# GithinjiHans/LZZX-NeRF

Measured on AMD Instinct MI355X. Metric: rendered samples/s (512x512 triplane head, max_steps 192), higher is better.
Workload: dtype f32

## Files before the change

### lzzx_nerf_amd/csrc/lz_frame.hip

```cpp
#include <stdlib.h>

#include "lz_march.h"
#include "lz_head_slice.h"
#include "lz_head_f16_slice.h"
#include "lz_head_f16w_slice.h"

#ifndef LZF_WG
#define LZF_WG 1024
#endif
#define LZF_WAVES (LZF_WG / 64)
#define LZF_BINS 256
#define LZF_LUT 256
#define LZF_MARCH_PROBES 2
#define LZF_Q_HEAD 0
#define LZF_Q_SIZE 1
#define LZF_DONE 3
#define LZF_SAMPLES 5
#define LZF_ITER 6
#define LZF_ROWS 72
#define LZF_P_HEAD 8
#define LZF_P_SIZE 9
#define LZF_CEFF 10
#define LZF_SCHED_K 11
#define LZF_TICKET 12
#define LZF_CAP_MAX_STEPS 4096
#define LZF_HIST 128
#define LZF_CURSOR 384

struct LzFrameK {
    const float* rays_o; const float* rays_d; const uint8_t* grid; const float* aabb;
    float* nears; float* fars; float* rays_t;
    int* order; int* state; uint8_t* keys;
    float* weights_sum; float* depth; float* image; float* amb0_sum; float* amb1_sum; float* unc_sum;
    float* out; const float* bg; uint8_t* out_rgb24; int* ray_counts;
    float bg_scalar, bound, dt_gamma, T_thresh, min_near;
    uint32_t N, max_steps, C, H;
    const float* noises;
    const float* occ;
    float* t_end;
    int* ray_last;
    int* cap_ws;
    uint32_t cap_mode, phase2, N_total;
    LzMarchFrame mf;
};

typedef const char __attribute__((address_space(4))) lz_kernarg_t;
struct LzfOut {
    lz_kernarg_t* f;
    template <typename T> __device__ __forceinline__ T get(size_t off) const {
        return *reinterpret_cast<const volatile T __attribute__((address_space(4)))*>(f + off);
    }
};
#define LZF_OUT(o, name) ((o).template get<decltype(LzFrameK::name)>(__builtin_offsetof(LzFrameK, name)))
static_assert(alignof(LzFrameK) == 8 && __is_trivially_copyable(LzFrameK), "LZF_OUT reads LzFrameK from the kernel-argument segment at round8(ARGS_BEFORE)");
template <size_t ARGS_BEFORE>
__device__ __forceinline__ LzfOut lzf_out() {
    return LzfOut{(lz_kernarg_t*)__builtin_amdgcn_kernarg_segment_ptr() + ((ARGS_BEFORE + 7) & ~size_t(7))};
}

__device__ __forceinline__ void lzf_write_pixel(const LzfOut& O, int ray, float ws, float d, float r, float g, float b, float a0, float a1,
                                                float u, int cnt) {
    LZF_OUT(O, weights_sum)[ray] = ws;
    LZF_OUT(O, depth)[ray] = d;
    const float rgb[3] = {r, g, b};
    float* image = LZF_OUT(O, image);
    float* out = LZF_OUT(O, out);
// ... 89 lines not shown
            const int v = (bin && threadIdx.x + off < LZF_BINS) ? start[threadIdx.x + off] : 0;
            __syncthreads();
            if (bin) start[threadIdx.x] += v;
            __syncthreads();
        }
        const int incl = bin ? start[threadIdx.x] : 0;
        __syncthreads();
        if (bin) start[threadIdx.x] = incl - h;
        if (blockIdx.x == 0 && threadIdx.x == 1) { F.state[LZF_Q_SIZE] = incl; F.state[LZF_DONE] = 1; F.state[LZF_ITER] = 1; }
    }
    __syncthreads();
    const uint32_t n = blockIdx.x * blockDim.x + threadIdx.x;
    const int key = n < F.N ? (int)F.keys[n] : 0;
    const int lrank = key > 0 ? atomicAdd(&lcount[key], 1) : 0;
    __syncthreads();
    if (bin && threadIdx.x > 0) {
        const int c = lcount[threadIdx.x];
        if (c > 0) lbase[threadIdx.x] = atomicAdd(F.state + LZF_CURSOR + threadIdx.x, c);
    }
    __syncthreads();
    if (key > 0) F.order[start[key] + lbase[key] + lrank] = (int)n;
}

enum { SF_RAY = 0, SF_T, SF_FAR, SF_DT, SF_WS, SF_D, SF_R, SF_G, SF_B, SF_A0, SF_A1, SF_U, SF_CNT,
       SF_SH };
template <int PREC, int S, int ROWS> struct LzfFields {
    static constexpr int SH_WORDS = PREC == 1 ? 8 : 16;
    static constexpr int ST = SF_SH + SH_WORDS;
    static constexpr int X = ST, Y = ST + 1, Z = ST + 2, TS = ST + 3;
    static constexpr int OSIG = S > 1 ? ST + 4 : ST, OR = OSIG + 1, OG = OSIG + 2, OB = OSIG + 3, OA0 = OSIG + 4, OA1 = OSIG + 5, OU = OSIG + 6;
    static constexpr int IT = OSIG + 7;
    static constexpr int RD = S > 1 ? ST + 12 : (ROWS > 1 ? ST + 7 : ST);
    static constexpr bool GEO = ROWS < 3;
    static constexpr int COUNT = RD + 3 + (GEO ? 6 : 0);
};

struct LzShFromSlot {
    const float* slot;
    int ls, ns;
    __device__ __forceinline__ void prepare() const {}
    __device__ __forceinline__ float comp_iq(int i, int q) const { return slot[(SF_SH + 4 * i + q) * ns + ls]; }
    __device__ __forceinline__ float comp_qj(int q, int j) const { return slot[(SF_SH + 4 * q + j) * ns + ls]; }
};
struct LzShFromSlot16 {
    const float* slot;
    int ls, ns;
    __device__ __forceinline__ void prepare() const {}
};
__device__ __forceinline__ void w_sh_pk(const LzShFromSlot16& f, int h, uint32_t (&w)[4]) {
#pragma unroll
    for (int k = 0; k < 4; k++) w[k] = __float_as_uint(f.slot[(SF_SH + 4 * h + k) * f.ns + f.ls]);
}
template <int PREC, bool GEO = false>
__device__ __forceinline__ void lzf_store_sh(const float* __restrict__ ro, const float* __restrict__ d, float* slot, int s, int ns, int rd_field) {
    float o[16];
    lz_sh_eval(d[0], d[1], d[2], 4, o, nullptr, nullptr, nullptr);
    slot[rd_field * ns + s] = 1 / d[0];
    slot[(rd_field + 1) * ns + s] = 1 / d[1];
    slot[(rd_field + 2) * ns + s] = 1 / d[2];
    if constexpr (GEO) {
#pragma unroll
        for (int k = 0; k < 3; k++) {
            slot[(rd_field + 3 + k) * ns + s] = ro[k];
            slot[(rd_field + 6 + k) * ns + s] = d[k];
        }
    }
    if constexpr (PREC == 1) {
#pragma unroll
        for (int k = 0; k < 8; k++) slot[(SF_SH + k) * ns + s] = __uint_as_float(h_cvt2(o[2 * k], o[2 * k + 1], false));
    } else {
#pragma unroll
        for (int k = 0; k < 16; k++) slot[(SF_SH + k) * ns + s] = o[k];
    }
}

__device__ __forceinline__ void lzf_slot_take(const LzfOut& O, bool ph2, int ray, float* slot, int* sloti, int sl, int ns) {
    if (__builtin_expect(ph2, 0)) {
        slot[SF_WS * ns + sl] = LZF_OUT(O, weights_sum)[ray];
        slot[SF_D * ns + sl] = LZF_OUT(O, depth)[ray];
        const float* image = LZF_OUT(O, image);
        slot[SF_R * ns + sl] = image[(size_t)ray * 3];
        slot[SF_G * ns + sl] = image[(size_t)ray * 3 + 1];
        slot[SF_B * ns + sl] = image[(size_t)ray * 3 + 2];
        slot[SF_A0 * ns + sl] = LZF_OUT(O, amb0_sum)[ray];
        slot[SF_A1 * ns + sl] = LZF_OUT(O, amb1_sum)[ray];
        slot[SF_U * ns + sl] = LZF_OUT(O, unc_sum)[ray];
        sloti[SF_CNT * ns + sl] = (int)LZF_OUT(O, max_steps);
    } else {
#pragma unroll
        for (int f = SF_WS; f <= SF_U; f++) slot[f * ns + sl] = 0.0f;
        sloti[SF_CNT * ns + sl] = 0;
    }
}
enum { LZF_END_BOX = 0, LZF_END_T = 1, LZF_END_CAP = 2 };
__device__ __forceinline__ void lzf_ray_end(const LzfOut& O, bool ph2, int ray, int kind, int composited, int report, float t, float ws, float d,
                                            float r, float g, float b, float a0, float a1, float u) {
    if (__builtin_expect(LZF_OUT(O, cap_mode) != 0, 0)) {
        report = composited;
        if (kind == LZF_END_T) {
            if (LZF_OUT(O, ray_counts)) { report = -composited; LZF_OUT(O, rays_t)[ray] = t; }
            if (!ph2) LZF_OUT(O, ray_last)[ray] = composited - 1;
        } else if (!ph2) {
            LZF_OUT(O, ray_last)[ray] = composited;
            if (kind == LZF_END_CAP) LZF_OUT(O, rays_t)[ray] = t;
        }
    }
    lzf_write_pixel(O, ray, ws, d, r, g, b, a0, a1, u, report);
}

template <int PREC> struct LzfHead;
template <> struct LzfHead<0> {
    using Args = LzHeadArgs; using Ctx = LzHeadCtx; using Out = LzHeadOut; using ShSlot = LzShFromSlot;
    static constexpr int LDS_WORDS = LzHeadLds<false>::FLOATS;
    __device__ static __forceinline__ void stage(const Args& P, float* lds, int q, Ctx& c) { lz_head_stage<false>(P, lds, LZF_WG, q, c); }
    template <typename ShFn>
    __device__ static __forceinline__ void slice(const Ctx& c, int lane, float x, float y, float z, ShFn f, Out& o) {
        lz_head_slice<false, false, true, true>(c, lane, x, y, z, f, o);
    }
};
template <> struct LzfHead<2> : LzfHead<0> {
    template <typename ShFn>
    __device__ static __forceinline__ void slice(const Ctx& c, int lane, float x, float y, float z, ShFn f, Out& o) {
        lz_head_slice<false, true, true, true>(c, lane, x, y, z, f, o);
    }
};
template <> struct LzfHead<1> {
    using Args = LzHead16Args; using Ctx = LzHead16Ctx; using Out = LzHead16wOut; using ShSlot = LzShFromSlot16;
    static constexpr int LDS_WORDS = LZ_HEAD16W_LDS_H8 * 4;
    __device__ static __forceinline__ void stage(const Args& P, float* lds, int, Ctx& c) { lz_head16w_stage(P, reinterpret_cast<lz_h8*>(lds), LZF_WG, c); }
    template <typename ShFn>
    __device__ static __forceinline__ void slice(const Ctx& c, int lane, float x, float y, float z, ShFn f, Out& o) {
        lz_head16w_slice<true, LZ_F16W_PRIO != 0>(c, lane, x, y, z, f, o);
    }
};

template <int PREC, int S, int ROWS>
__global__ void __launch_bounds__(LZF_WG, LZF_WG / 256)
lz_k_frame(typename LzfHead<PREC>::Args P, LzFrameK F) {
    using HD = LzfHead<PREC>;
    static_assert(PREC == 1 ? ROWS == 2 : (ROWS == 1 || S == 1), "slot rows per wave: f16 two; f32 one, or several with one sample per ray and pass");
    constexpr int NS = 16 * ROWS;
    using FL = LzfFields<PREC, S, ROWS>;
    constexpr int NF = FL::COUNT;
    constexpr int SF_X = FL::X, SF_Y = FL::Y, SF_Z = FL::Z, SF_TS = FL::TS, SF_OSIG = FL::OSIG, SF_OR = FL::OR, SF_OG = FL::OG, SF_OB = FL::OB,
                  SF_OA0 = FL::OA0, SF_OA1 = FL::OA1, SF_OU = FL::OU, SF_IT = FL::IT, SF_RD = FL::RD;
    (void)SF_RD; (void)SF_X; (void)SF_Y; (void)SF_Z; (void)SF_TS; (void)SF_IT; (void)SF_OSIG; (void)SF_OR; (void)SF_OG; (void)SF_OB; (void)SF_OA0; (void)SF_OA1; (void)SF_OU;
    constexpr int SLOT_WORDS = LZF_WAVES * NF * NS;
    __shared__ __align__(16) float lds[HD::LDS_WORDS + SLOT_WORDS + 4 + LZF_LUT];
    const int lane = threadIdx.x & 63, wave = threadIdx.x >> 6;
    const int s = (S > 1) ? (lane & (NS - 1)) : (lane & 15), q = lane >> 4;
    const bool slot_lane = lane < NS;
    static_assert(alignof(typename HD::Args) <= 8, "lz_k_frame(Args P, LzFrameK F): F sits at round8(sizeof(Args)) of the kernel-argument segment");
// ... 130 lines not shown
                            kk = got;
                            if (kk == 0) {
                                const int c0 = sloti[SF_CNT * NS + s];
                                lzf_ray_end(OUT, ph2, ray, LZF_END_BOX, c0, c0, t0, slot[SF_WS * NS + s], slot[SF_D * NS + s], slot[SF_R * NS + s], slot[SF_G * NS + s],
                                            slot[SF_B * NS + s], slot[SF_A0 * NS + s], slot[SF_A1 * NS + s], slot[SF_U * NS + s]);
                                my_samples += c0 - cnt_base;
                                ray = -1;
                                sloti[SF_RAY * NS + s] = -1;
                            }
                        }
                    }
                }
                if (!__ballot(leader && ray < 0 && !dry)) break;
            }
            if (leader) sloti[SF_IT * NS + s] = kk;
            if (!__ballot(kk > 0)) {
                if (dry) break;
                continue;
            }
            const int lkk = sloti[SF_IT * NS + lead];
            const bool live = sloti[SF_RAY * NS + lead] >= 0 && j < lkk;
            const float px = live ? slot[SF_X * NS + s] : 0.0f, py = live ? slot[SF_Y * NS + s] : 0.0f, pz = live ? slot[SF_Z * NS + s] : 0.0f;
            typename HD::Out o;
            HD::slice(ctx, lane, px, py, pz, typename HD::ShSlot{slot, lead, NS}, o);
            my_slices += ROWS;
            if constexpr (PREC == 1) {
                const int hh = lane >> 5;
                slot[(SF_OR + hh) * NS + s] = o.a;
                slot[(hh ? SF_OSIG : SF_OB) * NS + s] = hh ? 1.0f - lz_expf(-o.b * slot[SF_DT * NS + s]) : o.b;
                if (hh == 0) { slot[SF_OA0 * NS + s] = o.ambaud; slot[SF_OA1 * NS + s] = o.eyeatt; slot[SF_OU * NS + s] = o.unc; }
            } else if (q == 0) {
                slot[SF_OSIG * NS + s] = 1.0f - lz_expf(-o.sigma * slot[SF_DT * NS + s]);
                slot[SF_OR * NS + s] = o.rgb[0]; slot[SF_OG * NS + s] = o.rgb[1]; slot[SF_OB * NS + s] = o.rgb[2];
                slot[SF_OA0 * NS + s] = o.ambaud; slot[SF_OA1 * NS + s] = o.eyeatt; slot[SF_OU * NS + s] = o.unc;
            }
            __builtin_amdgcn_wave_barrier();
            if (leader && kk > 0) {
                float ws = slot[SF_WS * NS + s], d = slot[SF_D * NS + s], r = slot[SF_R * NS + s], g = slot[SF_G * NS + s], b = slot[SF_B * NS + s];
                float a0 = slot[SF_A0 * NS + s], a1 = slot[SF_A1 * NS + s], u = slot[SF_U * NS + s], t = slot[SF_T * NS + s];
                int step = 0;
                while (step < kk) {
                    const int sl = s + step;
                    const float alpha = slot[SF_OSIG * NS + sl];
                    const float T = 1 - ws;
                    const float w = alpha * T;
                    ws += w;
                    t = slot[SF_TS * NS + sl];
// ... 81 lines not shown
                        lzf_ray_end(OUT, ph2, ray, LZF_END_BOX, c0, c0, t, slot[SF_WS * NS + sl], slot[SF_D * NS + sl], slot[SF_R * NS + sl], slot[SF_G * NS + sl],
                                    slot[SF_B * NS + sl], slot[SF_A0 * NS + sl], slot[SF_A1 * NS + sl], slot[SF_U * NS + sl]);
                        my_samples += c0 - cnt_base;
                        ray = -1;
                        sloti[SF_RAY * NS + sl] = -1;
                        x = y = z = 0.0f;
                    }
                }
                if (!__ballot(slot_lane && ray < 0 && !dry)) break;
            }
            const unsigned long long have_mask = __ballot(have);
            if (!have_mask) {
                if (dry && !__ballot(slot_lane && ray >= 0)) break;
                continue;
            }
            typename HD::Out o;
            if constexpr (PREC == 1) {
                const int rs = lane & 31, hh = lane >> 5;
                auto lo2 = [](float v) -> float {
                    const auto r = __builtin_amdgcn_permlane32_swap(__float_as_uint(v), __float_as_uint(v), false, false);
                    return __uint_as_float(r[0]);
                };
                const float px = lo2(x), py = lo2(y), pz = lo2(z);
                HD::slice(ctx, lane, px, py, pz, typename HD::ShSlot{slot, rs, NS}, o);
                my_slices += 2;
                slot[(SF_OR + hh) * NS + rs] = o.a;
                slot[(hh ? SF_OSIG : SF_OB) * NS + rs] = o.b;
                if (hh == 0) { slot[SF_OA0 * NS + rs] = o.ambaud; slot[SF_OA1 * NS + rs] = o.eyeatt; slot[SF_OU * NS + rs] = o.unc; }
            } else {
#pragma unroll 1
                for (int row = 0; row < ROWS; row++) {
                    if (ROWS > 1 && !((have_mask >> (16 * row)) & 0xffffull)) continue;
                    const int rs = 16 * row + s;
                    const float px = __shfl(x, rs, 64), py = __shfl(y, rs, 64), pz = __shfl(z, rs, 64);
                    HD::slice(ctx, lane, px, py, pz, typename HD::ShSlot{slot, rs, NS}, o);
                    my_slices++;
                    if (ROWS > 1 && q == 0) {
                        slot[SF_OSIG * NS + rs] = o.sigma;
                        slot[SF_OR * NS + rs] = o.rgb[0]; slot[SF_OG * NS + rs] = o.rgb[1]; slot[SF_OB * NS + rs] = o.rgb[2];
                        slot[SF_OA0 * NS + rs] = o.ambaud; slot[SF_OA1 * NS + rs] = o.eyeatt; slot[SF_OU * NS + rs] = o.unc;
                    }
                }
            }
            __builtin_amdgcn_wave_barrier();
            if (have) {
                float sg, c0, c1, c2, am0, am1, un;
                if constexpr (PREC != 1) { sg = o.sigma; c0 = o.rgb[0]; c1 = o.rgb[1]; c2 = o.rgb[2]; am0 = o.ambaud; am1 = o.eyeatt; un = o.unc; }
                if (ROWS > 1) {
                    sg = slot[SF_OSIG * NS + sl];
                    c0 = slot[SF_OR * NS + sl]; c1 = slot[SF_OG * NS + sl]; c2 = slot[SF_OB * NS + sl];
                    am0 = slot[SF_OA0 * NS + sl]; am1 = slot[SF_OA1 * NS + sl]; un = slot[SF_OU * NS + sl];
                }
                const float dt = slot[SF_DT * NS + sl];
                float ws = slot[SF_WS * NS + sl];
                const float alpha = 1.0f - lz_expf(-sg * dt);
                const float T = 1 - ws;
                const float w = alpha * T;
                ws += w;
// ... 287 lines not shown
    return LZ_OK;
}

static void lzf_level_tables(const lz_head_params* p, float* scale, uint32_t* res) {
    for (int l = 0; l < 12; l++) {
        const float sc = exp2f((float)l * p->S) * (float)p->H - 1.0f;
        scale[l] = sc;
        res[l] = (uint32_t)ceilf(sc) + 1u;
    }
}

static int lzf_fill(const lz_frame_fused* f, LzFrameK& K) {
    K.rays_o = f->rays_o; K.rays_d = f->rays_d; K.grid = f->grid; K.aabb = f->aabb;
    K.nears = f->nears; K.fars = f->fars; K.rays_t = f->rays_t;
    K.order = f->order; K.state = f->state; K.keys = f->keys;
    K.weights_sum = f->weights_sum; K.depth = f->depth; K.image = f->image; K.amb0_sum = f->amb_aud_sum; K.amb1_sum = f->amb_eye_sum;
    K.unc_sum = f->unc_sum; K.out = f->out; K.bg = f->bg; K.out_rgb24 = f->out_rgb24; K.ray_counts = f->ray_counts;
    K.bg_scalar = f->bg_scalar; K.bound = f->bound; K.dt_gamma = f->dt_gamma; K.T_thresh = f->T_thresh; K.min_near = f->min_near;
    K.N = f->N; K.max_steps = f->max_steps; K.C = f->C; K.H = f->H;
    K.noises = f->noises;
    K.occ = f->occupied_aabb; K.t_end = f->t_end;
    K.ray_last = f->ray_last; K.cap_ws = f->cap_ws; K.cap_mode = f->cap_mode; K.phase2 = 0; K.N_total = f->N_total;
    K.mf = lz_march_frame(f->bound, f->max_steps, f->C, f->H);
    return LZ_OK;
}

static int lzf_check(const lz_frame_fused* f, const char* who) {
    const lz_head_params* p = &f->head;
    LZ_REQUIRE(f->rays_o && f->rays_d && f->grid && f->aabb && f->nears && f->fars && f->rays_t && f->order && f->state && f->keys &&
                   f->weights_sum && f->depth && f->image && f->amb_aud_sum && f->amb_eye_sum && f->unc_sum && f->out,
               LZ_ERR_BAD_ARGUMENT, "%s: incomplete lz_frame_fused", who);
    LZ_REQUIRE(p->emb_xy && p->emb_yz && p->emb_xz && p->offsets && p->packed && p->enc_a, LZ_ERR_BAD_ARGUMENT, "%s: incomplete lz_head_params", who);
    LZ_REQUIRE(p->testing, LZ_ERR_UNSUPPORTED, "%s: inference only (head.testing must be 1)", who);
    LZ_REQUIRE(p->precision >= 0 && p->precision <= 2, LZ_ERR_BAD_ARGUMENT, "%s: precision must be 0 (f32), 1 (f16) or 2 (f32, folded geo)", who);
    LZ_REQUIRE(f->C >= 1 && f->C <= 8 && f->H > 0, LZ_ERR_BAD_ARGUMENT, "%s: cascade must be in [1, 8]", who);
    LZ_REQUIRE(!f->occupied_aabb || f->t_end, LZ_ERR_BAD_ARGUMENT, "%s: occupied_aabb needs the t_end scratch buffer", who);
    LZ_REQUIRE(f->cap_mode == LZ_FRAME_CAP_PER_RAY || f->cap_mode == LZ_FRAME_CAP_REFERENCE, LZ_ERR_BAD_ARGUMENT, "%s: cap_mode must be 0 (per ray) or 1 (the reference's schedule)", who);
    if (f->cap_mode == LZ_FRAME_CAP_REFERENCE) {
        LZ_REQUIRE(f->ray_last && f->cap_ws, LZ_ERR_BAD_ARGUMENT, "%s: cap_mode 1 needs the ray_last and cap_ws buffers", who);
        LZ_REQUIRE(f->max_steps <= LZF_CAP_MAX_STEPS, LZ_ERR_UNSUPPORTED, "%s: cap_mode 1 supports max_steps <= %d", who, LZF_CAP_MAX_STEPS);
        LZ_REQUIRE(f->N_total == 0 || f->N_total >= f->N, LZ_ERR_BAD_ARGUMENT, "%s: N_total is the ray count of the whole frame (>= N)", who);
    }
    LZ_REQUIRE(f->bound > 0.0f && f->bound <= p->bound, LZ_ERR_BAD_ARGUMENT,
               "%s: the march's bound must not exceed the head's (the reference uses one `bound` for both, renderer.py:94, network.py:100)", who);
    return LZ_OK;
}
// ... 27 lines not shown
        a.offsets = p->offsets; a.packed = reinterpret_cast<const lz_h8*>(p->packed); a.enc_a = p->enc_a; a.ind_code = p->ind_code;
        a.eye = p->eye; a.bound = p->bound;
        lzf_level_tables(p, a.scale, a.res);
        switch (S) {
            case 1: hipLaunchKernelGGL((lz_k_frame<1, 1, 2>), dim3(grid), dim3(LZF_WG), 0, st, a, K); break;
            case 2: hipLaunchKernelGGL((lz_k_frame<1, 2, 2>), dim3(grid), dim3(LZF_WG), 0, st, a, K); break;
            case 4: hipLaunchKernelGGL((lz_k_frame<1, 4, 2>), dim3(grid), dim3(LZF_WG), 0, st, a, K); break;
            case 8: hipLaunchKernelGGL((lz_k_frame<1, 8, 2>), dim3(grid), dim3(LZF_WG), 0, st, a, K); break;
            default: hipLaunchKernelGGL((lz_k_frame<1, 16, 2>), dim3(grid), dim3(LZF_WG), 0, st, a, K); break;
        }
    } else {
        LzHeadArgs a;
        a.emb[0] = p->emb_xy; a.emb[1] = p->emb_yz; a.emb[2] = p->emb_xz;
        a.offsets = p->offsets; a.packed = reinterpret_cast<const float*>(p->packed); a.enc_a = p->enc_a; a.ind_code = p->ind_code; a.eye = p->eye;
        a.bound = p->bound; a.testing = 1;
        lzf_level_tables(p, a.scale, a.res);
        if (p->precision == 2) { LZF_SWITCH(2) } else { LZF_SWITCH(0) }
    }
#undef LZF_SWITCH
#undef LZF_LAUNCH
    return LZ_OK;
}

extern "C" int lz_frame_finish(const lz_frame_fused* f, lz_stream_t stream) {
    LZ_REQUIRE(f, LZ_ERR_BAD_ARGUMENT, "frame_finish: null");
    LZ_REQUIRE(f->cap_mode == LZ_FRAME_CAP_REFERENCE, LZ_ERR_BAD_ARGUMENT, "frame_finish: only after lz_frame_render with cap_mode 1");
    if (f->N == 0 && f->state) return LZ_OK;
    int rc = lzf_check(f, "frame_finish");
    if (rc != LZ_OK) return rc;
    hipStream_t st = lz_st(stream);
    LzFrameK K;
    lzf_fill(f, K);
    if (f->defer_finish) hipLaunchKernelGGL(lz_k_frame_schedule, dim3(1), dim3(256), LZF_SCHED_LDS_INTS(f->max_steps) * sizeof(int), st, K);
    K.phase2 = 1;
    rc = lzf_launch_persistent(f, K, st);
    if (rc != LZ_OK) return rc;
    if (f->ray_counts) hipLaunchKernelGGL(lz_k_frame_counts, dim3(lz_div_up(f->N, 256)), dim3(256), 0, st, K);
    LZ_CHECK_LAUNCH("frame_finish");
    return LZ_OK;
}

extern "C" int lz_frame_render(const lz_frame_fused* f, lz_timing* timing, lz_stream_t stream) {
    LZ_REQUIRE(f, LZ_ERR_BAD_ARGUMENT, "frame_render: null");
    hipStream_t st = lz_st(stream);
    if (f->N == 0 && f->state) {
        hipError_t e = hipMemsetAsync(f->state, 0, LZ_FRAME_STATE_INTS * sizeof(int32_t), st);
        if (e == hipSuccess && f->cap_mode == LZ_FRAME_CAP_REFERENCE && f->cap_ws) {
            LZ_REQUIRE(f->max_steps <= LZF_CAP_MAX_STEPS, LZ_ERR_UNSUPPORTED, "frame_render: cap_mode 1 supports max_steps <= %d", LZF_CAP_MAX_STEPS);
            e = hipMemsetAsync(f->cap_ws, 0, LZ_FRAME_CAP_WS_INTS((size_t)f->max_steps) * sizeof(int32_t), st);
        }
        if (e != hipSuccess) { lz_set_error("frame_render: memset: %s", hipGetErrorString(e)); return (int)e; }
        return LZ_OK;
    }
    int rc = lzf_check(f, "frame_render");
    if (rc != LZ_OK) return rc;
    LzFrameK K;
    lzf_fill(f, K);
    hipError_t hrc = hipMemsetAsync(f->state, 0, LZ_FRAME_STATE_INTS * sizeof(int32_t), st);
    if (hrc != hipSuccess) { lz_set_error("frame_render: memset: %s", hipGetErrorString(hrc)); return (int)hrc; }
    const bool ref_cap = f->cap_mode == LZ_FRAME_CAP_REFERENCE;
    const uint32_t nb = lz_div_up(f->N, LZF_PREP_WG);
    hipLaunchKernelGGL(lz_k_frame_prepare, dim3(nb), dim3(LZF_PREP_WG), 0, st, K);
    hipLaunchKernelGGL(lz_k_frame_scatter, dim3(nb), dim3(LZF_PREP_WG), 0, st, K);
    if (timing) (void)lz_timing_mark(timing, 0, stream);
    rc = lzf_launch_persistent(f, K, st);
    if (rc != LZ_OK) return rc;
    if (timing) (void)lz_timing_mark(timing, 1, stream);
    if (ref_cap) {
        const size_t lds = LZF_SCHED_LDS_INTS((size_t)f->max_steps) * sizeof(int);
        uint32_t hb = lz_div_up(f->N, 1024 * 8);
        hb = hb < 1 ? 1 : (hb > 32 ? 32 : hb);
        if (f->defer_finish) hipLaunchKernelGGL(lz_k_frame_cap_hist<false>, dim3(hb), dim3(1024), lds, st, K);
        else hipLaunchKernelGGL(lz_k_frame_cap_hist<true>, dim3(hb), dim3(1024), lds, st, K);
    }
    LZ_CHECK_LAUNCH("frame_render");
    if (ref_cap && !f->defer_finish) return lz_frame_finish(f, stream);
    return LZ_OK;
}
```

### lzzx_nerf_amd/csrc/lz_head_gather.h

```cpp
#ifndef LZ_HEAD_GATHER_H
#define LZ_HEAD_GATHER_H
#ifndef LZ_GATHER_PACK16
#define LZ_GATHER_PACK16 false
#endif
#ifndef LZ_GATHER_PACK32
#define LZ_GATHER_PACK32 false
#endif
#include "lz_common.h"
#include "lzzx_detmath.h"

#define LZ_LVTAB_WORDS 128
#define LZ_LVTAB_SCALE 16
#define LZ_LVTAB_STRIDE 32
#define LZ_LVTAB_QUEUE 48
#define LZ_LVTAB_HMUL 49
#define LZ_LVTAB_ENCA 64
#define LZ_LVTAB_MASK 96
#define LZ_LVTAB_ENCA16 108
#define LZ_LVTAB_IND16 124
#define LZ_LVTAB_DENSE0 62

__device__ __forceinline__ void lz_level_table_fill(int* tab, const int* __restrict__ offsets, const float* scale, const uint32_t* res) {
    const uint32_t t = threadIdx.x;
    if (t < 13) tab[t] = offsets[t];
    if (t < 12) {
        const uint32_t hs = (uint32_t)(offsets[t + 1] - offsets[t]), stride = res[t] + 1u;
        const bool dense = stride <= hs && (uint64_t)stride * stride <= hs;
        reinterpret_cast<float*>(tab)[LZ_LVTAB_SCALE + t] = scale[t];
        tab[LZ_LVTAB_STRIDE + t] = dense ? (int)stride : 0;
        tab[LZ_LVTAB_HMUL + t] = dense ? 0 : (int)(2654435761u & 0x00ffffffu);
        tab[LZ_LVTAB_MASK + t] = dense ? -1 : (int)(hs - 1u);
    }
    if (t == 0) {
        tab[LZ_LVTAB_QUEUE] = 0;
        int d0 = 1;
        for (int l = 0; l < 4; l++) {
// ... 144 lines not shown
```

### lzzx_nerf_amd/csrc/lz_head_layers.h

```cpp
#ifndef LZ_HEAD_LAYERS_H
#define LZ_HEAD_LAYERS_H
#include "lz_common.h"
#include "lzzx_detmath.h"

typedef float lz_f4 __attribute__((ext_vector_type(4)));

enum { LZ_L_A1 = 0, LZ_L_A2, LZ_L_E1, LZ_L_S1, LZ_L_S2, LZ_L_S3, LZ_L_C1, LZ_L_U1, LZ_L_COUNT };
constexpr int LZ_KS[LZ_L_COUNT] = {   9, 16,  9, 18, 16, 16, 21,  9 };
constexpr int LZ_NT[LZ_L_COUNT] = {   4,  2,  1,  4,  4,  4,  4,  2 };
constexpr int lz_frag_base(int layer) {
    int b = 0;
    for (int i = 0; i < layer; i++) b += LZ_KS[i] * LZ_NT[i];
    return b;
}
constexpr int lz_kt(int layer) { return (LZ_KS[layer] + 3) / 4; }
constexpr int lz_bfrag_base(int layer) {
    int b = 0;
    for (int i = 0; i < layer; i++) b += i == LZ_L_U1 ? 0 : lz_kt(i) * LZ_NT[i];
    return b;
}
constexpr int LZ_BFRAGS = lz_bfrag_base(LZ_L_COUNT);
constexpr int LZ_FRAGS_INFER = lz_frag_base(LZ_L_U1);
constexpr int LZ_FRAGS_ALL = lz_frag_base(LZ_L_COUNT);
constexpr int LZ_WV_C2 = 0, LZ_WV_SIG = 192, LZ_WV_E2 = 256, LZ_WV_U2 = 272, LZ_WV_FLOATS = 320;
static_assert(LZ_FRAGS_ALL * 64 + LZ_WV_FLOATS == LZ_HEAD_PACKED_FLOATS, "packed size mismatch with the header");


struct LzHeadArgs {
    const float* emb[3];
    const int* offsets;
    const float* packed;
    const float* enc_a;
    const float* ind_code;
    const float* eye;
    float bound;
    float scale[12];
    uint32_t res[12];
    int testing;
};

template <int LAYER, int T>
__device__ __forceinline__ void lz_layer(const float* __restrict__ wl, int lane, const float (&b)[T][LZ_KS[LAYER]],
                                         lz_f4 (&acc)[LZ_NT[LAYER]][T]) {
    constexpr int KS = LZ_KS[LAYER], NT = LZ_NT[LAYER];
    const float* frag = wl + lz_frag_base(LAYER) * 64 + lane;
#pragma unroll
    for (int ks = 0; ks < KS; ks++) {
        float a[NT];
#pragma unroll
        for (int ft = 0; ft < NT; ft++) a[ft] = frag[(ks * NT + ft) * 64];
#pragma unroll
        for (int ft = 0; ft < NT; ft++)
#pragma unroll
            for (int j = 0; j < T; j++) acc[ft][j] = __builtin_amdgcn_mfma_f32_16x16x4f32(a[ft], b[j][ks], acc[ft][j], 0, 0, 0);
    }
}

__device__ __forceinline__ float lz_relu(float v) { return v > 0.0f ? v : 0.0f; }

template <int NTILE>
__device__ __forceinline__ float lz_lane_dot(const float* __restrict__ wrow, int q, const float (&x)[4 * NTILE]) {
    float acc = 0.0f;
#pragma unroll
    for (int t = 0; t < NTILE; t++)
#pragma unroll
        for (int r = 0; r < 4; r++) acc = lz_fmaf(wrow[16 * t + 4 * q + r], x[4 * t + r], acc);
    acc += __shfl_xor(acc, 16, 64);
    acc += __shfl_xor(acc, 32, 64);
    return acc;
}

#endif
```

### lzzx_nerf_amd/csrc/lz_head_slice.h

```cpp
#ifndef LZ_HEAD_SLICE_H
#define LZ_HEAD_SLICE_H
#include "lz_common.h"
#include "lzzx_detmath.h"
#include "lzzx_sh_eval.h"
#include "lz_head_gather.h"
#include "lz_head_layers.h"

#define LZ_T 1

struct LzHeadCtx {
    const float* wl;
    const int* tab;
    const float* lenca;
    const float* emb[3];
    float bound, two_bound, eye_v, indq;
    bool has_eye;
};

struct LzHeadOut {
    float sigma, rgb[3], ambaud, eyeatt, unc;
};

template <bool TRAIN_UNC>
struct LzHeadLds {
    static constexpr int NFRAG = TRAIN_UNC ? LZ_FRAGS_ALL : LZ_FRAGS_INFER;
    static constexpr int WV = NFRAG * 64, TAB = WV + LZ_WV_FLOATS, FLOATS = TAB + LZ_LVTAB_WORDS;
};

template <bool TRAIN_UNC>
__device__ __forceinline__ void lz_head_stage(const LzHeadArgs& P, float* wl, uint32_t n_threads, int q, LzHeadCtx& hc) {
    using L = LzHeadLds<TRAIN_UNC>;
    const float4* src = reinterpret_cast<const float4*>(P.packed);
    float4* dst = reinterpret_cast<float4*>(wl);
    for (uint32_t i = threadIdx.x; i < (uint32_t)L::NFRAG * 16; i += n_threads) dst[i] = src[i];
    if (threadIdx.x < LZ_WV_FLOATS) wl[L::WV + threadIdx.x] = P.packed[LZ_FRAGS_ALL * 64 + threadIdx.x];
    int* tab = reinterpret_cast<int*>(wl + L::TAB);
    lz_level_table_fill(tab, P.offsets, P.scale, P.res);
    if (threadIdx.x < 32) wl[L::TAB + LZ_LVTAB_ENCA + threadIdx.x] = P.enc_a[threadIdx.x];
    hc.wl = wl;
    hc.tab = tab;
    hc.lenca = wl + L::TAB + LZ_LVTAB_ENCA;
    hc.emb[0] = P.emb[0]; hc.emb[1] = P.emb[1]; hc.emb[2] = P.emb[2];
    hc.bound = P.bound;
    hc.two_bound = 2.0f * P.bound;
    hc.has_eye = P.eye != nullptr;
    hc.eye_v = hc.has_eye ? P.eye[0] : 0.0f;
    hc.indq = P.ind_code ? P.ind_code[q] : 0.0f;
}

template <typename DirFn>
struct LzShFromDir {
    DirFn dirfn;
    float o[16];
    __device__ __forceinline__ explicit LzShFromDir(DirFn f) : dirfn(f) {}
    __device__ __forceinline__ void prepare() {
        float dx, dy, dz;
        dirfn(dx, dy, dz);
        lz_sh_eval(dx, dy, dz, 4, o, nullptr, nullptr, nullptr);
    }
    __device__ __forceinline__ float comp_iq(int i, int q) const {
        return q == 0 ? o[4 * i] : (q == 1 ? o[4 * i + 1] : (q == 2 ? o[4 * i + 2] : o[4 * i + 3]));
    }
    __device__ __forceinline__ float comp_qj(int q, int j) const {
        return q == 0 ? o[j] : (q == 1 ? o[4 + j] : (q == 2 ? o[8 + j] : o[12 + j]));
    }
};
template <typename DirFn>
__device__ __forceinline__ LzShFromDir<DirFn> lz_sh_from_dir(DirFn f) { return LzShFromDir<DirFn>(f); }

template <bool TRAIN_UNC, bool FOLD = false, bool IN_RANGE = false, bool YIELD = false, typename ShFn>
__device__ __forceinline__ void lz_head_slice(const LzHeadCtx& hc, int lane, float px, float py, float pz, ShFn shfn, LzHeadOut& out) {
    static_assert(!(TRAIN_UNC && FOLD), "the folded colour net is an inference arrangement");
    constexpr int WV = LzHeadLds<TRAIN_UNC>::WV;
    const int q = lane >> 4;
    float encx[LZ_T][9];
    lz_head_gather<IN_RANGE, LZ_GATHER_PACK32, YIELD, true>(hc.emb, hc.tab, px, py, pz, q, hc.bound, hc.two_bound, encx[0]);
    __builtin_amdgcn_sched_barrier(0);

    float att[LZ_T][8];
    {
        lz_f4 acc1[4][LZ_T];
#pragma unroll
        for (int ft = 0; ft < 4; ft++)
#pragma unroll
            for (int j = 0; j < LZ_T; j++) acc1[ft][j] = lz_f4{0, 0, 0, 0};
        lz_layer<LZ_L_A1, LZ_T>(hc.wl, lane, encx, acc1);
        float b2[LZ_T][16];
#pragma unroll
        for (int j = 0; j < LZ_T; j++)
#pragma unroll
            for (int ft = 0; ft < 4; ft++)
// ... 51 lines not shown
        for (int j = 0; j < LZ_T; j++)
#pragma unroll
            for (int ft = 0; ft < 2; ft++)
#pragma unroll
                for (int r = 0; r < 4; r++) bu[j][4 * ft + r] = lz_relu(accu[ft][j][r]);
#pragma unroll
        for (int j = 0; j < LZ_T; j++) uncv[j] = lz_softplusf(lz_lane_dot<2>(hc.wl + WV + LZ_WV_U2, q, bu[j]));
    } else {
#pragma unroll
        for (int j = 0; j < LZ_T; j++) uncv[j] = lz_softplusf(0.0f);
    }
    float geo[LZ_T][16];
    float sig_pre[LZ_T];
    {
        float b1[LZ_T][18];
#pragma unroll
        for (int j = 0; j < LZ_T; j++) {
#pragma unroll
            for (int i = 0; i < 9; i++) b1[j][i] = encx[j][i];
#pragma unroll
            for (int t = 0; t < 2; t++)
#pragma unroll
                for (int r = 0; r < 4; r++) b1[j][9 + 4 * t + r] = hc.lenca[16 * t + 4 * q + r] * att[j][4 * t + r];
            b1[j][17] = (hc.has_eye && q == 0) ? hc.eye_v * eyeatt[j] : 0.0f;
        }
        lz_f4 acc1[4][LZ_T];
#pragma unroll
        for (int ft = 0; ft < 4; ft++)
#pragma unroll
            for (int j = 0; j < LZ_T; j++) acc1[ft][j] = lz_f4{0, 0, 0, 0};
        lz_layer<LZ_L_S1, LZ_T>(hc.wl, lane, b1, acc1);
        float b2[LZ_T][16];
#pragma unroll
        for (int j = 0; j < LZ_T; j++)
#pragma unroll
            for (int ft = 0; ft < 4; ft++)
#pragma unroll
                for (int r = 0; r < 4; r++) b2[j][4 * ft + r] = lz_relu(acc1[ft][j][r]);
        lz_f4 acc2[4][LZ_T];
#pragma unroll
        for (int ft = 0; ft < 4; ft++)
#pragma unroll
            for (int j = 0; j < LZ_T; j++) acc2[ft][j] = lz_f4{0, 0, 0, 0};
        lz_layer<LZ_L_S2, LZ_T>(hc.wl, lane, b2, acc2);
        float b3[LZ_T][16];
#pragma unroll
        for (int j = 0; j < LZ_T; j++)
#pragma unroll
            for (int ft = 0; ft < 4; ft++)
#pragma unroll
                for (int r = 0; r < 4; r++) b3[j][4 * ft + r] = lz_relu(acc2[ft][j][r]);
        if constexpr (FOLD) {
#pragma unroll
            for (int j = 0; j < LZ_T; j++)
#pragma unroll
                for (int k = 0; k < 16; k++) geo[j][k] = b3[j][k];
        } else {
            lz_f4 acc3[4][LZ_T];
#pragma unroll
            for (int ft = 0; ft < 4; ft++)
#pragma unroll
                for (int j = 0; j < LZ_T; j++) acc3[ft][j] = lz_f4{0, 0, 0, 0};
            lz_layer<LZ_L_S3, LZ_T>(hc.wl, lane, b3, acc3);
#pragma unroll
            for (int j = 0; j < LZ_T; j++)
#pragma unroll
                for (int ft = 0; ft < 4; ft++)
#pragma unroll
                    for (int r = 0; r < 4; r++) geo[j][4 * ft + r] = acc3[ft][j][r];
        }
#pragma unroll
        for (int j = 0; j < LZ_T; j++) sig_pre[j] = lz_lane_dot<4>(hc.wl + WV + LZ_WV_SIG, q, b3[j]);
    }
    float rgb[LZ_T][3];
    {
        float b1[LZ_T][21];
#pragma unroll
        for (int j = 0; j < LZ_T; j++) {
            shfn.prepare();
#pragma unroll
            for (int i = 0; i < 4; i++) b1[j][i] = shfn.comp_iq(i, q);
#pragma unroll
            for (int k = 0; k < 16; k++) b1[j][4 + k] = geo[j][k];
            b1[j][20] = hc.indq;
        }
        lz_f4 acc1[4][LZ_T];
#pragma unroll
        for (int ft = 0; ft < 4; ft++)
#pragma unroll
            for (int j = 0; j < LZ_T; j++) acc1[ft][j] = lz_f4{0, 0, 0, 0};
        lz_layer<LZ_L_C1, LZ_T>(hc.wl, lane, b1, acc1);
        float b2[LZ_T][16];
#pragma unroll
        for (int j = 0; j < LZ_T; j++)
#pragma unroll
            for (int ft = 0; ft < 4; ft++)
#pragma unroll
                for (int r = 0; r < 4; r++) b2[j][4 * ft + r] = lz_relu(acc1[ft][j][r]);
#pragma unroll
        for (int j = 0; j < LZ_T; j++) {
            float d[3];
#pragma unroll
            for (int c = 0; c < 3; c++) d[c] = lz_lane_dot<4>(hc.wl + WV + LZ_WV_C2 + 64 * c, q, b2[j]);
            const float arg = q == 0 ? -d[0] : (q == 1 ? -d[1] : (q == 2 ? -d[2] : sig_pre[j]));
            const float e = lz_expf(arg);
            const float v = q == 3 ? e : (1.0f / (1.0f + e)) * 1.002f - 0.001f;
            const int s0 = lane & 15;
#pragma unroll
            for (int c = 0; c < 3; c++) rgb[j][c] = __shfl(v, s0 + 16 * c, 64);
            sig_pre[j] = __shfl(v, s0 + 48, 64);
        }
    }
    out.sigma = sig_pre[0];
    out.rgb[0] = rgb[0][0]; out.rgb[1] = rgb[0][1]; out.rgb[2] = rgb[0][2];
// ... 6 lines not shown
```

Measured before the change: 2.713 billion.

## Precompute per-ray SH color-layer partials and skip constant k-steps in head MFMAs

For the f32 head, a new kernel evaluates the SH-direction part of the first color layer once per ray and stores 64 floats per ray in a pooled buffer. The per-sample head loads that partial as its accumulator start and skips the SH k-steps, and the slot no longer holds 16 SH words, which shrinks LDS per slot. It also moves the eye and indicator k-steps out of the MFMA loops into VALU FMAs that run only when those inputs exist. The cost is an extra launch, a per-frame stream-ordered allocation, and global-memory reads of the partial inside the hot loop.

```diff
diff --git a/lzzx_nerf_amd/csrc/lz_frame.hip b/lzzx_nerf_amd/csrc/lz_frame.hip
--- a/lzzx_nerf_amd/csrc/lz_frame.hip
+++ b/lzzx_nerf_amd/csrc/lz_frame.hip
@@ -1,4 +1,6 @@
 #include <stdlib.h>
+
+#include <mutex>
 
 #include "lz_march.h"
 #include "lz_head_slice.h"
@@ -42,6 +44,7 @@
     int* cap_ws;
     uint32_t cap_mode, phase2, N_total;
     LzMarchFrame mf;
+    float* c1sh;
 };
 
 typedef const char __attribute__((address_space(4))) lz_kernarg_t;
@@ -177,10 +180,29 @@
     if (key > 0) F.order[start[key] + lbase[key] + lrank] = (int)n;
 }
 
+#define LZF_C1SH_WG 256
+__global__ void __launch_bounds__(LZF_C1SH_WG) lz_k_frame_c1sh(const float* __restrict__ packed, LzFrameK F) {
+    const int lane = threadIdx.x & 63, s = lane & 15, q = lane >> 4;
+    const int n_queue = F.state[F.phase2 ? LZF_P_SIZE : LZF_Q_SIZE];
+    const int tile = blockIdx.x * (LZF_C1SH_WG / 64) + (threadIdx.x >> 6);
+    if (tile * 16 >= n_queue) return;
+    const int idx = tile * 16 + s;
+    const int ray = idx < n_queue ? F.order[idx] : -1;
+    const float* d = F.rays_d + (size_t)(ray < 0 ? 0 : ray) * 3;
+    auto sh = lz_sh_from_dir([d](float& x, float& y, float& z) { x = d[0]; y = d[1]; z = d[2]; });
+    lz_f4 acc[4][1];
+    lz_c1_sh_partial(packed, lane, sh, acc);
+    if (ray >= 0) {
+        float* row = F.c1sh + (size_t)ray * LZ_C1_SH_FLOATS + 16 * q;
+#pragma unroll
+        for (int ft = 0; ft < 4; ft++) *reinterpret_cast<lz_f4*>(row + 4 * ft) = acc[ft][0];
+    }
+}
+
 enum { SF_RAY = 0, SF_T, SF_FAR, SF_DT, SF_WS, SF_D, SF_R, SF_G, SF_B, SF_A0, SF_A1, SF_U, SF_CNT,
        SF_SH };
 template <int PREC, int S, int ROWS> struct LzfFields {
-    static constexpr int SH_WORDS = PREC == 1 ? 8 : 16;
+    static constexpr int SH_WORDS = PREC == 1 ? 8 : 0;
     static constexpr int ST = SF_SH + SH_WORDS;
     static constexpr int X = ST, Y = ST + 1, Z = ST + 2, TS = ST + 3;
     static constexpr int OSIG = S > 1 ? ST + 4 : ST, OR = OSIG + 1, OG = OSIG + 2, OB = OSIG + 3, OA0 = OSIG + 4, OA1 = OSIG + 5, OU = OSIG + 6;
@@ -190,13 +212,6 @@
     static constexpr int COUNT = RD + 3 + (GEO ? 6 : 0);
 };
 
-struct LzShFromSlot {
-    const float* slot;
-    int ls, ns;
-    __device__ __forceinline__ void prepare() const {}
-    __device__ __forceinline__ float comp_iq(int i, int q) const { return slot[(SF_SH + 4 * i + q) * ns + ls]; }
-    __device__ __forceinline__ float comp_qj(int q, int j) const { return slot[(SF_SH + 4 * q + j) * ns + ls]; }
-};
 struct LzShFromSlot16 {
     const float* slot;
     int ls, ns;
@@ -208,8 +223,6 @@
 }
 template <int PREC, bool GEO = false>
 __device__ __forceinline__ void lzf_store_sh(const float* __restrict__ ro, const float* __restrict__ d, float* slot, int s, int ns, int rd_field) {
-    float o[16];
-    lz_sh_eval(d[0], d[1], d[2], 4, o, nullptr, nullptr, nullptr);
     slot[rd_field * ns + s] = 1 / d[0];
     slot[(rd_field + 1) * ns + s] = 1 / d[1];
     slot[(rd_field + 2) * ns + s] = 1 / d[2];
@@ -221,11 +234,10 @@
         }
     }
     if constexpr (PREC == 1) {
+        float o[16];
+        lz_sh_eval(d[0], d[1], d[2], 4, o, nullptr, nullptr, nullptr);
 #pragma unroll
         for (int k = 0; k < 8; k++) slot[(SF_SH + k) * ns + s] = __uint_as_float(h_cvt2(o[2 * k], o[2 * k + 1], false));
-    } else {
-#pragma unroll
-        for (int k = 0; k < 16; k++) slot[(SF_SH + k) * ns + s] = o[k];
     }
 }
 
@@ -265,9 +277,13 @@
 
 template <int PREC> struct LzfHead;
 template <> struct LzfHead<0> {
-    using Args = LzHeadArgs; using Ctx = LzHeadCtx; using Out = LzHeadOut; using ShSlot = LzShFromSlot;
+    using Args = LzHeadArgs; using Ctx = LzHeadCtx; using Out = LzHeadOut;
     static constexpr int LDS_WORDS = LzHeadLds<false>::FLOATS;
     __device__ static __forceinline__ void stage(const Args& P, float* lds, int q, Ctx& c) { lz_head_stage<false>(P, lds, LZF_WG, q, c); }
+    __device__ static __forceinline__ LzShPartial sh(const LzfOut& O, const float* slot, int ls, int ns, int q) {
+        const int ray = reinterpret_cast<const int*>(slot)[SF_RAY * ns + ls];
+        return LzShPartial{ray >= 0 ? LZF_OUT(O, c1sh) + (size_t)ray * LZ_C1_SH_FLOATS + 16 * q : nullptr};
+    }
     template <typename ShFn>
     __device__ static __forceinline__ void slice(const Ctx& c, int lane, float x, float y, float z, ShFn f, Out& o) {
         lz_head_slice<false, false, true, true>(c, lane, x, y, z, f, o);
@@ -280,9 +296,10 @@
     }
 };
 template <> struct LzfHead<1> {
-    using Args = LzHead16Args; using Ctx = LzHead16Ctx; using Out = LzHead16wOut; using ShSlot = LzShFromSlot16;
+    using Args = LzHead16Args; using Ctx = LzHead16Ctx; using Out = LzHead16wOut;
     static constexpr int LDS_WORDS = LZ_HEAD16W_LDS_H8 * 4;
     __device__ static __forceinline__ void stage(const Args& P, float* lds, int, Ctx& c) { lz_head16w_stage(P, reinterpret_cast<lz_h8*>(lds), LZF_WG, c); }
+    __device__ static __forceinline__ LzShFromSlot16 sh(const LzfOut&, const float* slot, int ls, int ns, int) { return LzShFromSlot16{slot, ls, ns}; }
     template <typename ShFn>
     __device__ static __forceinline__ void slice(const Ctx& c, int lane, float x, float y, float z, ShFn f, Out& o) {
         lz_head16w_slice<true, LZ_F16W_PRIO != 0>(c, lane, x, y, z, f, o);
@@ -459,7 +476,7 @@
             const bool live = sloti[SF_RAY * NS + lead] >= 0 && j < lkk;
             const float px = live ? slot[SF_X * NS + s] : 0.0f, py = live ? slot[SF_Y * NS + s] : 0.0f, pz = live ? slot[SF_Z * NS + s] : 0.0f;
             typename HD::Out o;
-            HD::slice(ctx, lane, px, py, pz, typename HD::ShSlot{slot, lead, NS}, o);
+            HD::slice(ctx, lane, px, py, pz, HD::sh(OUT, slot, lead, NS, q), o);
             my_slices += ROWS;
             if constexpr (PREC == 1) {
                 const int hh = lane >> 5;
@@ -587,7 +604,7 @@
                     return __uint_as_float(r[0]);
                 };
                 const float px = lo2(x), py = lo2(y), pz = lo2(z);
-                HD::slice(ctx, lane, px, py, pz, typename HD::ShSlot{slot, rs, NS}, o);
+                HD::slice(ctx, lane, px, py, pz, HD::sh(OUT, slot, rs, NS, q), o);
                 my_slices += 2;
                 slot[(SF_OR + hh) * NS + rs] = o.a;
                 slot[(hh ? SF_OSIG : SF_OB) * NS + rs] = o.b;
@@ -598,7 +615,7 @@
                     if (ROWS > 1 && !((have_mask >> (16 * row)) & 0xffffull)) continue;
                     const int rs = 16 * row + s;
                     const float px = __shfl(x, rs, 64), py = __shfl(y, rs, 64), pz = __shfl(z, rs, 64);
-                    HD::slice(ctx, lane, px, py, pz, typename HD::ShSlot{slot, rs, NS}, o);
+                    HD::slice(ctx, lane, px, py, pz, HD::sh(OUT, slot, rs, NS, q), o);
                     my_slices++;
                     if (ROWS > 1 && q == 0) {
                         slot[SF_OSIG * NS + rs] = o.sigma;
@@ -932,6 +949,45 @@
     K.occ = f->occupied_aabb; K.t_end = f->t_end;
     K.ray_last = f->ray_last; K.cap_ws = f->cap_ws; K.cap_mode = f->cap_mode; K.phase2 = 0; K.N_total = f->N_total;
     K.mf = lz_march_frame(f->bound, f->max_steps, f->C, f->H);
+    K.c1sh = nullptr;
+    return LZ_OK;
+}
+
+static hipMemPool_t lzf_c1sh_pool() {
+    static std::mutex mu;
+    static hipMemPool_t pools[64] = {};
+    int dev = 0;
+    if (hipGetDevice(&dev) != hipSuccess || dev < 0 || dev >= 64) return nullptr;
+    std::lock_guard<std::mutex> lock(mu);
+    if (!pools[dev]) {
+        hipMemPoolProps props;
+        memset(&props, 0, sizeof(props));
+        props.allocType = hipMemAllocationTypePinned;
+        props.location.type = hipMemLocationTypeDevice;
+        props.location.id = dev;
+        hipMemPool_t pool = nullptr;
+        if (hipMemPoolCreate(&pool, &props) != hipSuccess) return nullptr;
+        uint64_t keep = UINT64_MAX;
+        (void)hipMemPoolSetAttribute(pool, hipMemPoolAttrReleaseThreshold, &keep);
+        pools[dev] = pool;
+    }
+    return pools[dev];
+}
+struct LzfC1Sh {
+    float* p = nullptr;
+    hipStream_t st = nullptr;
+    ~LzfC1Sh() { if (p) (void)hipFreeAsync(p, st); }
+};
+static int lzf_c1sh_prepare(const lz_frame_fused* f, LzFrameK& K, LzfC1Sh& buf, hipStream_t st) {
+    if (f->head.precision == 1) return LZ_OK;
+    hipMemPool_t pool = lzf_c1sh_pool();
+    LZ_REQUIRE(pool, (int)hipErrorNotSupported, "frame_render: no memory pool for the SH partials");
+    const hipError_t e = hipMallocFromPoolAsync(reinterpret_cast<void**>(&buf.p), (size_t)f->N * LZ_C1_SH_FLOATS * sizeof(float), pool, st);
+    if (e != hipSuccess) { buf.p = nullptr; lz_set_error("frame_render: SH partials: %s", hipGetErrorString(e)); return (int)e; }
+    buf.st = st;
+    K.c1sh = buf.p;
+    hipLaunchKernelGGL(lz_k_frame_c1sh, dim3(lz_div_up(f->N, 16 * (LZF_C1SH_WG / 64))), dim3(LZF_C1SH_WG), 0, st,
+                       reinterpret_cast<const float*>(f->head.packed), K);
     return LZ_OK;
 }
 
@@ -1005,22 +1061,29 @@
     return LZ_OK;
 }
 
+static int lzf_finish(const lz_frame_fused* f, hipStream_t st, float* c1sh) {
+    LzFrameK K;
+    lzf_fill(f, K);
+    if (f->defer_finish) hipLaunchKernelGGL(lz_k_frame_schedule, dim3(1), dim3(256), LZF_SCHED_LDS_INTS(f->max_steps) * sizeof(int), st, K);
+    K.phase2 = 1;
+    LzfC1Sh own;
+    int rc = LZ_OK;
+    if (c1sh) K.c1sh = c1sh;
+    else if ((rc = lzf_c1sh_prepare(f, K, own, st)) != LZ_OK) return rc;
+    rc = lzf_launch_persistent(f, K, st);
+    if (rc != LZ_OK) return rc;
+    if (f->ray_counts) hipLaunchKernelGGL(lz_k_frame_counts, dim3(lz_div_up(f->N, 256)), dim3(256), 0, st, K);
+    LZ_CHECK_LAUNCH("frame_finish");
+    return LZ_OK;
+}
+
 extern "C" int lz_frame_finish(const lz_frame_fused* f, lz_stream_t stream) {
     LZ_REQUIRE(f, LZ_ERR_BAD_ARGUMENT, "frame_finish: null");
     LZ_REQUIRE(f->cap_mode == LZ_FRAME_CAP_REFERENCE, LZ_ERR_BAD_ARGUMENT, "frame_finish: only after lz_frame_render with cap_mode 1");
     if (f->N == 0 && f->state) return LZ_OK;
     int rc = lzf_check(f, "frame_finish");
     if (rc != LZ_OK) return rc;
-    hipStream_t st = lz_st(stream);
-    LzFrameK K;
-    lzf_fill(f, K);
-    if (f->defer_finish) hipLaunchKernelGGL(lz_k_frame_schedule, dim3(1), dim3(256), LZF_SCHED_LDS_INTS(f->max_steps) * sizeof(int), st, K);
-    K.phase2 = 1;
-    rc = lzf_launch_persistent(f, K, st);
-    if (rc != LZ_OK) return rc;
-    if (f->ray_counts) hipLaunchKernelGGL(lz_k_frame_counts, dim3(lz_div_up(f->N, 256)), dim3(256), 0, st, K);
-    LZ_CHECK_LAUNCH("frame_finish");
-    return LZ_OK;
+    return lzf_finish(f, lz_st(stream), nullptr);
 }
 
 extern "C" int lz_frame_render(const lz_frame_fused* f, lz_timing* timing, lz_stream_t stream) {
@@ -1045,6 +1108,9 @@
     const uint32_t nb = lz_div_up(f->N, LZF_PREP_WG);
     hipLaunchKernelGGL(lz_k_frame_prepare, dim3(nb), dim3(LZF_PREP_WG), 0, st, K);
     hipLaunchKernelGGL(lz_k_frame_scatter, dim3(nb), dim3(LZF_PREP_WG), 0, st, K);
+    LzfC1Sh c1sh;
+    rc = lzf_c1sh_prepare(f, K, c1sh, st);
+    if (rc != LZ_OK) return rc;
     if (timing) (void)lz_timing_mark(timing, 0, stream);
     rc = lzf_launch_persistent(f, K, st);
     if (rc != LZ_OK) return rc;
@@ -1057,6 +1123,6 @@
         else hipLaunchKernelGGL(lz_k_frame_cap_hist<true>, dim3(hb), dim3(1024), lds, st, K);
     }
     LZ_CHECK_LAUNCH("frame_render");
-    if (ref_cap && !f->defer_finish) return lz_frame_finish(f, stream);
+    if (ref_cap && !f->defer_finish) return lzf_finish(f, st, c1sh.p);
     return LZ_OK;
 }
diff --git a/lzzx_nerf_amd/csrc/lz_head_gather.h b/lzzx_nerf_amd/csrc/lz_head_gather.h
--- a/lzzx_nerf_amd/csrc/lz_head_gather.h
+++ b/lzzx_nerf_amd/csrc/lz_head_gather.h
@@ -12,6 +12,7 @@
 #define LZ_LVTAB_WORDS 128
 #define LZ_LVTAB_SCALE 16
 #define LZ_LVTAB_STRIDE 32
+#define LZ_LVTAB_IND 44
 #define LZ_LVTAB_QUEUE 48
 #define LZ_LVTAB_HMUL 49
 #define LZ_LVTAB_ENCA 64
diff --git a/lzzx_nerf_amd/csrc/lz_head_layers.h b/lzzx_nerf_amd/csrc/lz_head_layers.h
--- a/lzzx_nerf_amd/csrc/lz_head_layers.h
+++ b/lzzx_nerf_amd/csrc/lz_head_layers.h
@@ -39,13 +39,14 @@
     int testing;
 };
 
-template <int LAYER, int T>
-__device__ __forceinline__ void lz_layer(const float* __restrict__ wl, int lane, const float (&b)[T][LZ_KS[LAYER]],
-                                         lz_f4 (&acc)[LZ_NT[LAYER]][T]) {
-    constexpr int KS = LZ_KS[LAYER], NT = LZ_NT[LAYER];
+template <int LAYER, int T, int K0, int K1>
+__device__ __forceinline__ void lz_layer_ks(const float* __restrict__ wl, int lane, const float (&b)[T][LZ_KS[LAYER]],
+                                            lz_f4 (&acc)[LZ_NT[LAYER]][T]) {
+    constexpr int NT = LZ_NT[LAYER];
+    static_assert(0 <= K0 && K0 <= K1 && K1 <= LZ_KS[LAYER], "k-step range");
     const float* frag = wl + lz_frag_base(LAYER) * 64 + lane;
 #pragma unroll
-    for (int ks = 0; ks < KS; ks++) {
+    for (int ks = K0; ks < K1; ks++) {
         float a[NT];
 #pragma unroll
         for (int ft = 0; ft < NT; ft++) a[ft] = frag[(ks * NT + ft) * 64];
@@ -54,6 +55,11 @@
 #pragma unroll
             for (int j = 0; j < T; j++) acc[ft][j] = __builtin_amdgcn_mfma_f32_16x16x4f32(a[ft], b[j][ks], acc[ft][j], 0, 0, 0);
     }
+}
+template <int LAYER, int T>
+__device__ __forceinline__ void lz_layer(const float* __restrict__ wl, int lane, const float (&b)[T][LZ_KS[LAYER]],
+                                         lz_f4 (&acc)[LZ_NT[LAYER]][T]) {
+    lz_layer_ks<LAYER, T, 0, LZ_KS[LAYER]>(wl, lane, b, acc);
 }
 
 __device__ __forceinline__ float lz_relu(float v) { return v > 0.0f ? v : 0.0f; }
diff --git a/lzzx_nerf_amd/csrc/lz_head_slice.h b/lzzx_nerf_amd/csrc/lz_head_slice.h
--- a/lzzx_nerf_amd/csrc/lz_head_slice.h
+++ b/lzzx_nerf_amd/csrc/lz_head_slice.h
@@ -14,7 +14,8 @@
     const float* lenca;
     const float* emb[3];
     float bound, two_bound, eye_v, indq;
-    bool has_eye;
+    const float* lind;
+    bool has_eye, has_ind;
 };
 
 struct LzHeadOut {
@@ -46,13 +47,18 @@
     hc.has_eye = P.eye != nullptr;
     hc.eye_v = hc.has_eye ? P.eye[0] : 0.0f;
     hc.indq = P.ind_code ? P.ind_code[q] : 0.0f;
+    hc.has_ind = P.ind_code != nullptr;
+    if (threadIdx.x < 4) wl[L::TAB + LZ_LVTAB_IND + threadIdx.x] = P.ind_code ? P.ind_code[threadIdx.x] : 0.0f;
+    hc.lind = wl + L::TAB + LZ_LVTAB_IND;
 }
 
 template <typename DirFn>
 struct LzShFromDir {
     DirFn dirfn;
     float o[16];
+    static constexpr bool C1_PARTIAL = false;
     __device__ __forceinline__ explicit LzShFromDir(DirFn f) : dirfn(f) {}
+    __device__ __forceinline__ void issue(int) {}
     __device__ __forceinline__ void prepare() {
         float dx, dy, dz;
         dirfn(dx, dy, dz);
@@ -67,6 +73,30 @@
 };
 template <typename DirFn>
 __device__ __forceinline__ LzShFromDir<DirFn> lz_sh_from_dir(DirFn f) { return LzShFromDir<DirFn>(f); }
+
+constexpr int LZ_C1_SH_KS = 4;
+constexpr int LZ_C1_SH_FLOATS = 64;
+template <typename ShFn>
+__device__ __forceinline__ void lz_c1_sh_partial(const float* __restrict__ wl, int lane, ShFn& sh, lz_f4 (&acc)[4][1]) {
+    const int q = lane >> 4;
+    float b[1][LZ_KS[LZ_L_C1]];
+    sh.prepare();
+#pragma unroll
+    for (int i = 0; i < LZ_KS[LZ_L_C1]; i++) b[0][i] = i < LZ_C1_SH_KS ? sh.comp_iq(i, q) : 0.0f;
+#pragma unroll
+    for (int ft = 0; ft < 4; ft++) acc[ft][0] = lz_f4{0, 0, 0, 0};
+    lz_layer_ks<LZ_L_C1, 1, 0, LZ_C1_SH_KS>(wl, lane, b, acc);
+}
+struct LzShPartial {
+    static constexpr bool C1_PARTIAL = true;
+    const float* row;
+    lz_f4 p[4];
+    __device__ __forceinline__ void issue(int) {
+#pragma unroll
+        for (int ft = 0; ft < 4; ft++) p[ft] = row ? *reinterpret_cast<const lz_f4*>(row + 4 * ft) : lz_f4{0, 0, 0, 0};
+    }
+    __device__ __forceinline__ lz_f4 part(int ft) const { return p[ft]; }
+};
 
 template <bool TRAIN_UNC, bool FOLD = false, bool IN_RANGE = false, bool YIELD = false, typename ShFn>
 __device__ __forceinline__ void lz_head_slice(const LzHeadCtx& hc, int lane, float px, float py, float pz, ShFn shfn, LzHeadOut& out) {
@@ -164,14 +194,27 @@
             for (int t = 0; t < 2; t++)
 #pragma unroll
                 for (int r = 0; r < 4; r++) b1[j][9 + 4 * t + r] = hc.lenca[16 * t + 4 * q + r] * att[j][4 * t + r];
-            b1[j][17] = (hc.has_eye && q == 0) ? hc.eye_v * eyeatt[j] : 0.0f;
+            b1[j][17] = 0.0f;
         }
         lz_f4 acc1[4][LZ_T];
 #pragma unroll
         for (int ft = 0; ft < 4; ft++)
 #pragma unroll
             for (int j = 0; j < LZ_T; j++) acc1[ft][j] = lz_f4{0, 0, 0, 0};
-        lz_layer<LZ_L_S1, LZ_T>(hc.wl, lane, b1, acc1);
+        lz_layer_ks<LZ_L_S1, LZ_T, 0, 17>(hc.wl, lane, b1, acc1);
+        if (hc.has_eye) {
+            const float* w68 = hc.wl + (lz_frag_base(LZ_L_S1) + 17 * LZ_NT[LZ_L_S1]) * 64 + 4 * q;
+#pragma unroll
+            for (int j = 0; j < LZ_T; j++) {
+                const float e = hc.eye_v * eyeatt[j];
+#pragma unroll
+                for (int ft = 0; ft < 4; ft++) {
+                    const lz_f4 w = *reinterpret_cast<const lz_f4*>(w68 + 64 * ft);
+#pragma unroll
+                    for (int r = 0; r < 4; r++) acc1[ft][j][r] = lz_fmaf(w[r], e, acc1[ft][j][r]);
+                }
+            }
+        }
         float b2[LZ_T][16];
 #pragma unroll
         for (int j = 0; j < LZ_T; j++)
@@ -179,6 +222,7 @@
             for (int ft = 0; ft < 4; ft++)
 #pragma unroll
                 for (int r = 0; r < 4; r++) b2[j][4 * ft + r] = lz_relu(acc1[ft][j][r]);
+        shfn.issue(q);
         lz_f4 acc2[4][LZ_T];
 #pragma unroll
         for (int ft = 0; ft < 4; ft++)
@@ -216,22 +260,42 @@
     }
     float rgb[LZ_T][3];
     {
+        constexpr bool IND_VALU = !FOLD;
         float b1[LZ_T][21];
+        lz_f4 acc1[4][LZ_T];
 #pragma unroll
         for (int j = 0; j < LZ_T; j++) {
-            shfn.prepare();
-#pragma unroll
-            for (int i = 0; i < 4; i++) b1[j][i] = shfn.comp_iq(i, q);
+            if constexpr (ShFn::C1_PARTIAL) {
+#pragma unroll
+                for (int i = 0; i < LZ_C1_SH_KS; i++) b1[j][i] = 0.0f;
+#pragma unroll
+                for (int ft = 0; ft < 4; ft++) acc1[ft][j] = shfn.part(ft);
+            } else {
+                shfn.prepare();
+#pragma unroll
+                for (int i = 0; i < 4; i++) b1[j][i] = shfn.comp_iq(i, q);
+#pragma unroll
+                for (int ft = 0; ft < 4; ft++) acc1[ft][j] = lz_f4{0, 0, 0, 0};
+            }
 #pragma unroll
             for (int k = 0; k < 16; k++) b1[j][4 + k] = geo[j][k];
-            b1[j][20] = hc.indq;
-        }
-        lz_f4 acc1[4][LZ_T];
-#pragma unroll
-        for (int ft = 0; ft < 4; ft++)
-#pragma unroll
-            for (int j = 0; j < LZ_T; j++) acc1[ft][j] = lz_f4{0, 0, 0, 0};
-        lz_layer<LZ_L_C1, LZ_T>(hc.wl, lane, b1, acc1);
+            b1[j][20] = IND_VALU ? 0.0f : hc.indq;
+        }
+        lz_layer_ks<LZ_L_C1, LZ_T, ShFn::C1_PARTIAL ? LZ_C1_SH_KS : 0, LZ_KS[LZ_L_C1] - (IND_VALU ? 1 : 0)>(hc.wl, lane, b1, acc1);
+        if (IND_VALU && hc.has_ind) {
+            const float* w80 = hc.wl + (lz_frag_base(LZ_L_C1) + 20 * LZ_NT[LZ_L_C1]) * 64 + 4 * q;
+            const lz_f4 ind = *reinterpret_cast<const lz_f4*>(hc.lind);
+#pragma unroll
+            for (int j = 0; j < LZ_T; j++)
+#pragma unroll
+                for (int k = 0; k < 4; k++)
+#pragma unroll
+                    for (int ft = 0; ft < 4; ft++) {
+                        const lz_f4 w = *reinterpret_cast<const lz_f4*>(w80 + 64 * ft + 16 * k);
+#pragma unroll
+                        for (int r = 0; r < 4; r++) acc1[ft][j][r] = lz_fmaf(w[r], ind[k], acc1[ft][j][r]);
+                    }
+        }
         float b2[LZ_T][16];
 #pragma unroll
         for (int j = 0; j < LZ_T; j++)
```

Result: faster. 2.805 billion, median of 6 (+3.4%).
